# Onr/Council-GAN

Hardware: NVIDIA H100
Metric: training images/sec (gen+dis step) (higher is better)
Workload: dtype tf32

## Files before the change

### council_gan_b200/csrc/api.cu

```cuda
#include "common.cuh"
#include <string.h>

namespace cg {

static thread_local char g_err[512] = "";
std::atomic<uint64_t> g_launches{0};
thread_local int g_tc_mode = 7;
thread_local int g_pdl = 0;

void set_error(const char* fmt, ...) {
    va_list ap;
    va_start(ap, fmt);
    vsnprintf(g_err, sizeof(g_err), fmt, ap);
    va_end(ap);
}

int validate_geom(const cg_conv_geom& g) {
    CG_REQUIRE(g.G >= 1 && (g.x_groups == 1 || g.x_groups == g.G), "conv: x_groups=%d must be 1 or G=%d", g.x_groups, g.G);
    CG_REQUIRE(g.Cin % 4 == 0 && g.Cin > 0, "conv: Cin=%d must be a positive multiple of 4", g.Cin);
    CG_REQUIRE(g.Cout > 0 && g.B > 0 && g.H > 0 && g.W > 0, "conv: empty tensor");
    CG_REQUIRE(g.stride >= 1 && g.KH >= 1 && g.KW >= 1 && g.pad >= 0, "conv: bad kernel geometry");
    int Hin = g.ups ? 2 * g.H : g.H, Win = g.ups ? 2 * g.W : g.W;
    int Ho = (Hin + 2 * g.pad - g.KH) / g.stride + 1, Wo = (Win + 2 * g.pad - g.KW) / g.stride + 1;
    CG_REQUIRE(Ho == g.Ho && Wo == g.Wo, "conv: output size %dx%d inconsistent with geometry (expected %dx%d)", g.Ho, g.Wo, Ho, Wo);
// ... 52 lines not shown
    if (dir == 0) {
        if (i >= rows * K2p) return;
        long r = i / K2p;
        int k = (int)(i - r * K2p);
        dst[i] = k < K2 ? __ldg(src + r * K2 + k) : 0.f;
    } else {
        if (i >= rows * K2) return;
        long r = i / K2;
        int k = (int)(i - r * K2);
        dst[i] = __ldg(src + r * K2p + k);
    }
}
static int run_im2col(const cg_conv_geom& g, const float* x, float* P, cudaStream_t st) {
    cg_conv_geom p = patch_geom(g);
    long nimg = (long)(g.x_groups == 1 ? 1 : g.G) * g.B;
    long total4 = nimg * g.Ho * g.Wo * (p.Cin / 4);
    launch_k(im2col_small_kernel, cdiv(total4, 256), 256, 0, st, x, P, total4, g.H, g.W, g.Cin, g.Ho, g.Wo, g.KH, g.KW, g.stride, g.pad,
                                                          g.KH * g.KW * g.Cin, p.Cin);
    return check_launch("im2col_small");
}

}

using namespace cg;

extern "C" const char* cg_last_error(void) { return g_err; }

extern "C" int cg_device_info(int* sm_count, int* cc_major, int* cc_minor) {
    int dev = 0;
    cudaError_t e = cudaGetDevice(&dev);
    if (e != cudaSuccess) {
        set_error("cudaGetDevice: %s", cudaGetErrorString(e));
        return CG_ERR_NO_DEVICE;
    }
    cudaDeviceProp prop;
    e = cudaGetDeviceProperties(&prop, dev);
    if (e != cudaSuccess) {
        set_error("cudaGetDeviceProperties: %s", cudaGetErrorString(e));
        return CG_ERR_NO_DEVICE;
    }
    if (sm_count) *sm_count = prop.multiProcessorCount;
    if (cc_major) *cc_major = prop.major;
    if (cc_minor) *cc_minor = prop.minor;
    return prop.multiProcessorCount;
}

extern "C" int cg_set_tensor_core_mode(int mode) {
    int prev = g_tc_mode;
    g_tc_mode = mode == 1 ? 7 : (mode & 7);
    g_small_bn = ((mode >> 23) & 1) ? 0 : 1;
    g_wgrad_tma = ((mode >> 25) & 1) ? 0 : 1;
    g_pdl = (mode >> 22) & 1;
    g_tc_serial_epilogue = (mode >> 26) & 1;
    return prev;
}

extern "C" uint64_t cg_launch_count(void) { return g_launches.load(); }
extern "C" void cg_tensor_map_cache_stats(uint64_t* hits, uint64_t* misses) { tc_map_cache_stats(hits, misses); }

extern "C" int cg_zero(void* ptr, size_t bytes, void* stream) {
    cudaError_t e = cudaMemsetAsync(ptr, 0, bytes, (cudaStream_t)stream);
    if (e != cudaSuccess) {
        set_error("cg_zero: %s", cudaGetErrorString(e));
        return CG_ERR_CUDA;
    }
    return CG_OK;
}

extern "C" size_t cg_conv_workspace_bytes(const cg_conv_geom* g, int which) {
    if (!g) return 0;
    ConvDims d = conv_dims(*g);
    size_t need = 0;
    const bool patch_fwd = which == 0 && (g_tc_mode & 1) && patch_path(*g) && g->KH * g->KW >= 16;
    if (which == 2 && small_wgrad_supported(*g)) return small_ws(*g, 2);
    if (which == 1 && small_dgrad_supported(*g)) return small_ws(*g, 1);
    const bool patch_wgrad = which == 2 && (g_tc_mode & 4) && patch_path(*g);
    if (patch_fwd || patch_wgrad) {
        cg_conv_geom p = patch_geom(*g);
        ConvDims dp = conv_dims(p);
        size_t inner = which == 2 ? tc_wgrad_ws(p) : 0;
        size_t cs = which == 2 ? colsum_ws(g->G, dp.Mpix, g->Cout) : 0;
        if (cs > inner) inner = cs;
        need = patch_bytes(*g) + 2 * patch_w_bytes(*g) + inner;
        if (which == 2) return need;
    }
    if (which == 0 && (g_tc_mode & 1) && tc_fwd_supported(*g)) { size_t t = tc_fwd_ws(*g); need = t > need ? t : need; }
    if (which == 1) {
        if (g->ups) need = (size_t)g->G * g->B * d.Hin * d.Win * g->Cin * sizeof(float);
        if ((g_tc_mode & 2) && tc_dgrad_supported(*g)) { size_t t = tc_dgrad_ws(*g); need = t > need ? t : need; }
    }
    if (which == 2) {
        size_t a = ((g_tc_mode & 4) && tc_wgrad_supported(*g)) ? tc_wgrad_ws(*g) : simt_wgrad_ws(*g);
        size_t b = colsum_ws(g->G, d.Mpix, g->Cout);
        need = a > b ? a : b;
    }
    return need;
}

extern "C" int cg_conv_fwd(const cg_conv_geom* g, const float* x, const float* w, const float* bias, float* y, int act,
                           float slope, void* ws, size_t ws_bytes, void* stream) {
    if (int rc = validate_geom(*g)) return rc;
    cudaStream_t st = (cudaStream_t)stream;
    if (small_fwd_supported(*g, act)) return small_conv_fwd(*g, x, w, bias, y, st);
    if ((g_tc_mode & 1) && patch_path(*g) && g->KH * g->KW >= 16 && act != CG_ACT_TANH) {
        size_t need = cg_conv_workspace_bytes(g, 0);
        if (need > ws_bytes) {
// ... 108 lines not shown
```

### council_gan_b200/csrc/common.cuh

```cuda
#pragma once
#include <cuda.h>
#include <cuda_runtime.h>
#include <stdint.h>
#include <stdio.h>
#include <stdarg.h>
#include <atomic>
#include "../../include/council_b200.h"

namespace cg {

void set_error(const char* fmt, ...);
extern std::atomic<uint64_t> g_launches;
extern thread_local int g_tc_mode;
extern thread_local int g_small_bn;
extern thread_local int g_wgrad_tma;
extern thread_local int g_tc_serial_epilogue;

constexpr int CG_MAX_DEVICES = 64;
inline int current_device() {
    int dev = 0;
    cudaGetDevice(&dev);
    return dev >= 0 && dev < CG_MAX_DEVICES ? dev : 0;
}
struct PerDeviceOnce {
    std::atomic<bool> done[CG_MAX_DEVICES];
    bool first() { return !done[current_device()].exchange(true); }
    void reset() { done[current_device()].store(false); }
};

inline int check_launch(const char* what) {
    g_launches.fetch_add(1, std::memory_order_relaxed);
    cudaError_t e = cudaGetLastError();
    if (e != cudaSuccess) {
        set_error("%s: %s", what, cudaGetErrorString(e));
        return CG_ERR_CUDA;
    }
    return CG_OK;
}

#define CG_REQUIRE(cond, ...)                \
    do {                                     \
        if (!(cond)) {                       \
            cg::set_error(__VA_ARGS__);      \
            return CG_ERR_ARG;               \
        }                                    \
    } while (0)

static inline int cdiv(long a, long b) { return (int)((a + b - 1) / b); }

extern thread_local int g_pdl;
__device__ __forceinline__ void pdl_trigger() { asm volatile("griddepcontrol.launch_dependents;" ::: "memory"); }
__device__ __forceinline__ void pdl_wait() { asm volatile("griddepcontrol.wait;" ::: "memory"); }

template <typename... KArgs, typename... Args>
inline void launch_k(void (*kern)(KArgs...), dim3 grid, dim3 block, size_t smem, cudaStream_t st, Args&&... args) {
    cudaLaunchConfig_t cfg = {};
    cfg.gridDim = grid;
    cfg.blockDim = block;
    cfg.dynamicSmemBytes = smem;
    cfg.stream = st;
    cudaLaunchAttribute at[1];
    at[0].id = cudaLaunchAttributeProgrammaticStreamSerialization;
    at[0].val.programmaticStreamSerializationAllowed = g_pdl;
    cfg.attrs = at;
    cfg.numAttrs = 1;
    (void)cudaLaunchKernelEx(&cfg, kern, static_cast<KArgs>(args)...);
}

__device__ __forceinline__ float apply_act(float v, int act, float slope) {
// ... 63 lines not shown
```

### council_gan_b200/csrc/conv_tc.cu

```cuda
#include "common.cuh"
#include "tc_ptx.cuh"
#include <cstdlib>
#include <cstdio>
#include <cuda.h>
#include <mutex>
#include <string.h>

namespace cg {

typedef CUresult (*EncodeTiledFn)(CUtensorMap*, CUtensorMapDataType, cuuint32_t, void*, const cuuint64_t*, const cuuint64_t*,
                                  const cuuint32_t*, const cuuint32_t*, CUtensorMapInterleave, CUtensorMapSwizzle,
                                  CUtensorMapL2promotion, CUtensorMapFloatOOBfill);
typedef CUresult (*EncodeIm2colFn)(CUtensorMap*, CUtensorMapDataType, cuuint32_t, void*, const cuuint64_t*, const cuuint64_t*,
                                   const int*, const int*, cuuint32_t, cuuint32_t, const cuuint32_t*, CUtensorMapInterleave,
                                   CUtensorMapSwizzle, CUtensorMapL2promotion, CUtensorMapFloatOOBfill);
static EncodeTiledFn g_encode_tiled = nullptr;
static EncodeIm2colFn g_encode_im2col = nullptr;
static int g_sm_count_dev[CG_MAX_DEVICES] = {0};
static int sm_count_now() {
    int dev = current_device();
    if (!g_sm_count_dev[dev]) cudaDeviceGetAttribute(&g_sm_count_dev[dev], cudaDevAttrMultiProcessorCount, dev);
    return g_sm_count_dev[dev];
}
thread_local int g_small_bn = 1;
thread_local int g_tc_serial_epilogue = 0;
static int g_driver_version = 0;
static std::once_flag g_once;

struct MapKey {
    const void* ptr;
    int64_t a, b;
    int32_t v[8];
    bool operator==(const MapKey& o) const { return ptr == o.ptr && a == o.a && b == o.b && memcmp(v, o.v, sizeof(v)) == 0; }
};
struct MapSlot {
    MapKey key;
    CUtensorMap map;
    bool used;
};
constexpr int MAP_SLOTS = 8192;
static MapSlot* g_map_cache = nullptr;
static std::mutex g_map_mutex;
static std::atomic<uint64_t> g_map_hits{0}, g_map_misses{0};
static inline uint32_t map_hash(const MapKey& k) {
    uint64_t h = 1469598103934665603ull;
    const unsigned char* p = reinterpret_cast<const unsigned char*>(&k);
    for (size_t i = 0; i < sizeof(MapKey); i++) h = (h ^ p[i]) * 1099511628211ull;
    return (uint32_t)(h ^ (h >> 32)) & (MAP_SLOTS - 1);
}
template <class F>
static int cached_map(CUtensorMap* out, const MapKey& key, F encode) {
    const uint32_t slot = map_hash(key);
    {
        std::lock_guard<std::mutex> lock(g_map_mutex);
        if (!g_map_cache) g_map_cache = new MapSlot[MAP_SLOTS]();
        MapSlot& s = g_map_cache[slot];
        if (s.used && s.key == key) {
            *out = s.map;
            g_map_hits.fetch_add(1, std::memory_order_relaxed);
            return CG_OK;
        }
    }
    if (int rc = encode(out)) return rc;
    g_map_misses.fetch_add(1, std::memory_order_relaxed);
    std::lock_guard<std::mutex> lock(g_map_mutex);
    MapSlot& s = g_map_cache[slot];
    s.key = key;
    s.map = *out;
    s.used = true;
    return CG_OK;
}
void tc_map_cache_stats(uint64_t* hits, uint64_t* misses) {
    *hits = g_map_hits.load();
    *misses = g_map_misses.load();
}

static void init_driver() {
    std::call_once(g_once, [] {
        cudaDriverEntryPointQueryResult q;
        void* fn = nullptr;
        if (cudaGetDriverEntryPoint("cuTensorMapEncodeTiled", &fn, cudaEnableDefault, &q) == cudaSuccess && q == cudaDriverEntryPointSuccess)
            g_encode_tiled = (EncodeTiledFn)fn;
        fn = nullptr;
        if (cudaGetDriverEntryPoint("cuTensorMapEncodeIm2col", &fn, cudaEnableDefault, &q) == cudaSuccess && q == cudaDriverEntryPointSuccess)
            g_encode_im2col = (EncodeIm2colFn)fn;
        cudaDriverGetVersion(&g_driver_version);
    });
}

constexpr int TC_BM = 128;
constexpr int TC_BK = 32;
constexpr int TC_THREADS = 384;
constexpr int TC_MAX_STAGES = 12;
constexpr int TC_MAX_CLASSES = 4;

struct TcClass {
    CUtensorMap amap;
    int w0, h0;
    int out_h0, out_w0;
    int wrow_off;
    int pad_;
};
struct TcParams {
    CUtensorMap bmap;
    TcClass cls[TC_MAX_CLASSES];
    int ncls;
    int G, xg_images;
    int B, P, Q;
    int Cin, Cout, KH, KW, stride;
    int bn;
    int bk;
    int cps;
    int n_store;
    int out_H, out_W, out_sh, out_sw;
    int w_rows_per_group;
    float* y; const float* bias; const float* addend; const float* mask_src;
    float* stats;
    long stats_gbc;
    int act; float slope;
    int stages;
    int serial_epilogue;
};

__device__ __forceinline__ void tc_tile(const TcParams& p, int t, int MT, int NT, int& mt, int& nt, int& c, int& g) {
    if (p.serial_epilogue) {
        mt = t % MT;
        int r = t / MT;
        nt = r % NT;
        r /= NT;
        c = r % p.ncls;
        g = r / p.ncls;
        return;
    }
    c = t % p.ncls;
    int r = t / p.ncls;
    mt = r % MT;
    r /= MT;
    nt = r % NT;
    g = r / NT;
}

template <int BK, int BN>
__global__ void __launch_bounds__(TC_THREADS, 1) conv_tc_kernel(const __grid_constant__ TcParams p) {
    pdl_trigger();
    extern __shared__ __align__(1024) uint8_t smem_raw[];
    uint8_t* smem = reinterpret_cast<uint8_t*>((reinterpret_cast<uintptr_t>(smem_raw) + 1023) & ~(uintptr_t)1023);
    const int wg = __shfl_sync(0xffffffffu, threadIdx.x >> 7, 0), tid = threadIdx.x & 127;
    constexpr int a_bytes = TC_BM * BK * 4;
    constexpr int b_bytes = ((BN * BK * 4) + 1023) & ~1023;
    const int stage_bytes = p.cps * (a_bytes + b_bytes);
    constexpr int tx_chunk = a_bytes + BN * BK * 4;
    uint64_t* full_bar = reinterpret_cast<uint64_t*>(smem + (size_t)p.stages * stage_bytes);
    uint64_t* empty_bar = full_bar + p.stages;

    const int MT = (p.B * p.P * p.Q + TC_BM - 1) / TC_BM;
    const int NT = (p.Cout + BN - 1) / BN;
    const int tiles = p.G * p.ncls * NT * MT;
    const int kchunks = (p.Cin + BK - 1) / BK;
    const int kiters = p.KH * p.KW * kchunks;

    if (threadIdx.x == 0) {
        prefetch_tmap(&p.bmap);
        for (int c = 0; c < p.ncls; c++) prefetch_tmap(&p.cls[c].amap);
        for (int s = 0; s < p.stages; s++) {
            mbar_init(&full_bar[s], 1);
            mbar_init(&empty_bar[s], 2);
        }
        fence_barrier_init();
    }
    __syncthreads();
    pdl_wait();

    if (wg == 0) {
        if (tid == 0) {
            int stage = 0;
            uint32_t phase = 0;
            for (int t = blockIdx.x; t < tiles; t += gridDim.x) {
                int mt, nt, c, g;
                tc_tile(p, t, MT, NT, mt, nt, c, g);
                const TcClass& cl = p.cls[c];
                long m0 = (long)mt * TC_BM;
                int img = (int)(m0 / (p.P * p.Q));
                int rem = (int)(m0 - (long)img * p.P * p.Q);
                int pp = rem / p.Q, qq = rem - pp * p.Q;
                int n_coord = g * p.xg_images + img;
                int w_coord = cl.w0 + qq * p.stride;
                int h_coord = cl.h0 + pp * p.stride;
                int wrow = g * p.w_rows_per_group + cl.wrow_off + nt * BN;
                int kh = 0, kw = 0, kc = 0;
                for (int k0 = 0; k0 < kiters; k0 += p.cps) {
                    const int n = kiters - k0 < p.cps ? kiters - k0 : p.cps;
                    mbar_wait(&empty_bar[stage], phase ^ 1);
                    uint8_t* sa = smem + (size_t)stage * stage_bytes;
                    uint8_t* sb = sa + p.cps * a_bytes;
                    mbar_expect_tx(&full_bar[stage], (uint32_t)(n * tx_chunk));
                    for (int j = 0; j < n; j++) {
                        tma_load_im2col_4d(&cl.amap, &full_bar[stage], sa + j * a_bytes, kc * BK, w_coord, h_coord, n_coord, (uint16_t)kw,
                                           (uint16_t)kh);
                        tma_load_2d(&p.bmap, &full_bar[stage], sb + j * b_bytes, (kh * p.KW + kw) * p.Cin + kc * BK, wrow);
                        if (++kc == kchunks) { kc = 0; if (++kw == p.KW) { kw = 0; ++kh; } }
                    }
                    if (++stage == p.stages) { stage = 0; phase ^= 1; }
                }
            }
        }
        return;
    }

    const int cw = wg - 1;
    const int warp4 = tid >> 5, lane = tid & 31;
    const int row0 = cw * 64 + warp4 * 16 + (lane >> 2);
    const int cq = 2 * (lane & 3);
    const uint64_t desc0 = BK == 32 ? make_kmajor_sw128_desc(0) : make_kmajor_sw32_desc(0);
    float acc[BN / 2];
    int stage = 0;
    uint32_t phase = 0;
    for (int t = blockIdx.x; t < tiles; t += gridDim.x) {
        int mt, nt, c, g;
        tc_tile(p, t, MT, NT, mt, nt, c, g);
        const TcClass& cl = p.cls[c];
        int prev = -1;
        for (int k0 = 0; k0 < kiters; k0 += p.cps) {
            const int n = kiters - k0 < p.cps ? kiters - k0 : p.cps;
            mbar_wait(&full_bar[stage], phase);
            const uint32_t sa = smem_u32(smem + (size_t)stage * stage_bytes) + cw * (64 * BK * 4);
            const uint32_t sb = smem_u32(smem + (size_t)stage * stage_bytes) + p.cps * a_bytes;
            wgmma_fence();
            for (int j = 0; j < n; j++) {
                const uint64_t adesc = desc0 | (uint64_t)(((sa + j * a_bytes) & 0x3FFFF) >> 4);
                const uint64_t bdesc = desc0 | (uint64_t)(((sb + j * b_bytes) & 0x3FFFF) >> 4);
#pragma unroll
                for (int kk = 0; kk < BK / 8; kk++)
                    wgmma_tf32<BN>(acc, adesc + (uint64_t)(kk * 2), bdesc + (uint64_t)(kk * 2), (k0 | j | kk) != 0 ? 1 : 0);
            }
            wgmma_commit();
            wgmma_wait<1>();
            if (prev >= 0 && tid == 0) mbar_arrive(&empty_bar[prev]);
            prev = stage;
            if (++stage == p.stages) { stage = 0; phase ^= 1; }
        }
        wgmma_wait<0>();
        wgmma_reg_fence(acc, BN / 2);
        if (tid == 0) mbar_arrive(&empty_bar[prev]);

        const int pq = p.P * p.Q;
        long out_off[2];
        bool valid[2];
#pragma unroll
        for (int h = 0; h < 2; h++) {
            const int m = mt * TC_BM + row0 + 8 * h;
            valid[h] = m < p.B * pq;
            out_off[h] = 0;
            if (valid[h]) {
                int img = m / pq;
                int rem = m - img * pq;
                int pp = rem / p.Q, qq = rem - pp * p.Q;
                long pix = ((long)(g * p.B + img) * p.out_H + (pp * p.out_sh + cl.out_h0)) * p.out_W + (qq * p.out_sw + cl.out_w0);
                out_off[h] = pix * p.Cout + nt * p.n_store;
            }
        }
        if (p.stats) {
            const int tiles_per_img = pq / TC_BM;
            const int img = (mt * TC_BM) / pq;
            const int chunk = ((c * tiles_per_img + (mt - img * tiles_per_img)) << 3) + cw * 4 + warp4;
            const bool b2 = lane & 4, b3 = lane & 8;
            float* st = p.stats + ((long)chunk * p.stats_gbc + (long)(g * p.B + img) * p.Cout + nt * BN + cq) * 2 + (b3 ? 2 : 0) + (b2 ? 1 : 0);
#pragma unroll
            for (int j = 0; j < BN / 8; j++) {
                const float s0 = acc[4 * j] + acc[4 * j + 2], s1 = acc[4 * j + 1] + acc[4 * j + 3];
                const float q0 = acc[4 * j] * acc[4 * j] + acc[4 * j + 2] * acc[4 * j + 2];
                const float q1 = acc[4 * j + 1] * acc[4 * j + 1] + acc[4 * j + 3] * acc[4 * j + 3];
                const float k0 = b2 ? q0 : s0, k1 = b2 ? q1 : s1;
                const float r0 = __shfl_xor_sync(0xffffffffu, b2 ? s0 : q0, 4), r1 = __shfl_xor_sync(0xffffffffu, b2 ? s1 : q1, 4);
                const float x0 = k0 + r0, x1 = k1 + r1;
                float v = (b3 ? x1 : x0) + __shfl_xor_sync(0xffffffffu, b3 ? x0 : x1, 8);
                v += __shfl_xor_sync(0xffffffffu, v, 16);
                if (lane < 16) st[16 * j] = v;
            }
        }
        if (!(p.addend || p.mask_src) || p.serial_epilogue) {
#pragma unroll
            for (int j = 0; j < BN / 8; j++) {
                const int col = 8 * j + cq;
                if (col >= p.n_store) break;
                float2 bv = make_float2(0.f, 0.f);
                if (p.bias) bv = __ldg(reinterpret_cast<const float2*>(p.bias + (long)g * p.Cout + nt * p.n_store + col));
#pragma unroll
                for (int h = 0; h < 2; h++) {
                    if (!valid[h]) continue;
                    float2 o = make_float2(acc[4 * j + 2 * h] + bv.x, acc[4 * j + 2 * h + 1] + bv.y);
                    if (p.addend) {
                        const float2 a = __ldg(reinterpret_cast<const float2*>(p.addend + out_off[h] + col));
                        o.x += a.x; o.y += a.y;
                    }
                    if (p.mask_src) {
                        const float2 a = __ldg(reinterpret_cast<const float2*>(p.mask_src + out_off[h] + col));
                        o.x *= a.x > 0.f ? 1.f : p.slope; o.y *= a.y > 0.f ? 1.f : p.slope;
                    } else if (p.act != CG_ACT_NONE) {
                        o.x = apply_act(o.x, p.act, p.slope); o.y = apply_act(o.y, p.act, p.slope);
                    }
                    *reinterpret_cast<float2*>(p.y + out_off[h] + col) = o;
                }
            }
            continue;
        }
        constexpr int EB = BN == 256 ? 2 : BN / 8 < 8 ? BN / 8 : 8;
#pragma unroll
        for (int j0 = 0; j0 < BN / 8; j0 += EB) {
            float2 av[EB][2], mv[EB][2];
#pragma unroll
            for (int jj = 0; jj < EB; jj++) {
                const int col = 8 * (j0 + jj) + cq;
#pragma unroll
                for (int h = 0; h < 2; h++) {
                    const bool ld = col < p.n_store && valid[h];
                    av[jj][h] = p.addend && ld ? __ldg(reinterpret_cast<const float2*>(p.addend + out_off[h] + col)) : make_float2(0.f, 0.f);
                    mv[jj][h] = p.mask_src && ld ? __ldg(reinterpret_cast<const float2*>(p.mask_src + out_off[h] + col)) : make_float2(0.f, 0.f);
                }
            }
#pragma unroll
            for (int jj = 0; jj < EB; jj++) {
                const int j = j0 + jj, col = 8 * j + cq;
#pragma unroll
                for (int h = 0; h < 2; h++) {
                    if (col >= p.n_store || !valid[h]) continue;
                    float2 o = make_float2(acc[4 * j + 2 * h] + 0.f, acc[4 * j + 2 * h + 1] + 0.f);
                    if (p.addend) { o.x += av[jj][h].x; o.y += av[jj][h].y; }
                    if (p.mask_src) { o.x *= mv[jj][h].x > 0.f ? 1.f : p.slope; o.y *= mv[jj][h].y > 0.f ? 1.f : p.slope; }
                    *reinterpret_cast<float2*>(p.y + out_off[h] + col) = o;
                }
            }
        }
    }
}


static int encode_weights_map_raw(CUtensorMap* map, const float* w, long rows, long ktot, int bn, int bk) {
    cuuint64_t dims[2] = {(cuuint64_t)ktot, (cuuint64_t)rows};
    cuuint64_t strides[1] = {(cuuint64_t)ktot * 4};
    cuuint32_t box[2] = {(cuuint32_t)bk, (cuuint32_t)bn};
    cuuint32_t estr[2] = {1, 1};
    CUresult r = g_encode_tiled(map, CU_TENSOR_MAP_DATA_TYPE_TFLOAT32, 2, (void*)w, dims, strides, box, estr,
                                CU_TENSOR_MAP_INTERLEAVE_NONE, bk == 32 ? CU_TENSOR_MAP_SWIZZLE_128B : CU_TENSOR_MAP_SWIZZLE_32B,
                                CU_TENSOR_MAP_L2_PROMOTION_L2_256B, CU_TENSOR_MAP_FLOAT_OOB_FILL_NONE);
    if (r != CUDA_SUCCESS) {
        set_error("cuTensorMapEncodeTiled(weights rows=%ld ktot=%ld bn=%d) failed: %d", rows, ktot, bn, (int)r);
        return CG_ERR_CUDA;
    }
    return CG_OK;
}

static int encode_weights_map(CUtensorMap* map, const float* w, long rows, long ktot, int bn, int bk = TC_BK) {
    MapKey k{};
    k.ptr = w; k.a = rows; k.b = ktot; k.v[0] = bn; k.v[1] = bk; k.v[7] = 1;
    return cached_map(map, k, [&](CUtensorMap* m) { return encode_weights_map_raw(m, w, rows, ktot, bn, bk); });
}

static int encode_weights_map_p(TcParams& p, const float* w, long rows, long ktot) {
    return encode_weights_map(&p.bmap, w, rows, ktot, p.bn, p.bk);
}

static int encode_act_map_raw(CUtensorMap* map, const float* x, long N, int H, int W, int C, int lo_w, int lo_h, int up_w, int up_h,
                              int stride, int bk) {
    cuuint64_t dims[4] = {(cuuint64_t)C, (cuuint64_t)W, (cuuint64_t)H, (cuuint64_t)N};
    cuuint64_t strides[3] = {(cuuint64_t)C * 4, (cuuint64_t)W * C * 4, (cuuint64_t)H * W * C * 4};
    int lower[2] = {lo_w, lo_h};
    int upper[2] = {up_w, up_h};
    cuuint32_t estr[4] = {1, (cuuint32_t)stride, (cuuint32_t)stride, 1};
    CUresult r = g_encode_im2col(map, CU_TENSOR_MAP_DATA_TYPE_TFLOAT32, 4, (void*)x, dims, strides, lower, upper, bk, TC_BM, estr,
                                 CU_TENSOR_MAP_INTERLEAVE_NONE, bk == 32 ? CU_TENSOR_MAP_SWIZZLE_128B : CU_TENSOR_MAP_SWIZZLE_32B,
                                 CU_TENSOR_MAP_L2_PROMOTION_L2_128B, CU_TENSOR_MAP_FLOAT_OOB_FILL_NONE);
    if (r != CUDA_SUCCESS) {
        set_error("cuTensorMapEncodeIm2col(N=%ld H=%d W=%d C=%d corners %d,%d / %d,%d stride %d) failed: %d", N, H, W, C, lo_w, lo_h,
                  up_w, up_h, stride, (int)r);
        return CG_ERR_CUDA;
    }
    if (g_driver_version <= 13010 && (long)N * H * W * C * 4 < 131072) reinterpret_cast<uint64_t*>(map)[1] &= ~(1ull << 21);
    return CG_OK;
}

static int encode_act_map(CUtensorMap* map, const float* x, long N, int H, int W, int C, int lo_w, int lo_h, int up_w, int up_h,
                          int stride, int bk = TC_BK) {
    MapKey k{};
    k.ptr = x; k.a = N; k.b = ((int64_t)H << 32) | (uint32_t)W;
    k.v[0] = C; k.v[1] = lo_w; k.v[2] = lo_h; k.v[3] = up_w; k.v[4] = up_h; k.v[5] = stride; k.v[6] = bk; k.v[7] = 2;
    return cached_map(map, k, [&](CUtensorMap* m) { return encode_act_map_raw(m, x, N, H, W, C, lo_w, lo_h, up_w, up_h, stride, bk); });
}

static int pick_bn(int cout) {
    if (cout % 256 == 0) return 256;
    if (cout == 128) return 128;
    if (cout == 64) return 64;
    if (cout <= 16 && cout % 4 == 0) return 16;
    return 0;
}
static int pick_bk(int cin) {
    if (cin % TC_BK == 0) return TC_BK;
    if (cin <= 16 && cin % 4 == 0) return 8;
    return 0;
}

static int fill_bn(int bn, long mpix, int groups_classes, int cout) {
    if (!g_small_bn) return bn;
    const int sms = sm_count_now();
    while (bn > 64 && cout % (bn / 2) == 0 && (long)groups_classes * cdiv(mpix, TC_BM) * (cout / bn) < sms) bn >>= 1;
    return bn;
}

bool tc_fwd_supported(const cg_conv_geom& g) {
    init_driver();
    if (!g_encode_tiled || !g_encode_im2col) return false;
    if (g.ups && !(g.KH == 3 && g.KW == 3 && g.stride == 1 && g.pad == 1 && g.Cin % TC_BK == 0)) return false;
    if (pick_bk(g.Cin) == 0) return false;
    if (pick_bn(g.Cout) == 0) return false;
    if (g.pad > 120 || g.KH > 120) return false;
    if ((long)g.B * (g.ups ? g.H * g.W : g.Ho * g.Wo) < TC_BM) return false;
    return true;
}

template <int BK>
static void (*tc_kernel_for(int bn))(TcParams) {
    switch (bn) {
        case 16: return conv_tc_kernel<BK, 16>;
        case 64: return conv_tc_kernel<BK, 64>;
        case 128: return conv_tc_kernel<BK, 128>;
        case 256: return conv_tc_kernel<BK, 256>;
    }
    return nullptr;
}

static int launch_tc(TcParams& p, cudaStream_t st) {
    int a_bytes = TC_BM * p.bk * 4, b_bytes = ((p.bn * p.bk * 4) + 1023) & ~1023;
    int chunk_bytes = a_bytes + b_bytes;
    int kiters = p.KH * p.KW * ((p.Cin + p.bk - 1) / p.bk);
    int cps = p.bn <= 128 ? 2 : 1;
    if (p.bk == 8) cps = 8;
    while (cps > 1 && (cps > kiters || cps * chunk_bytes > 64 * 1024)) cps >>= 1;
    p.cps = cps;
    int stage_bytes = cps * chunk_bytes;
    int stages = (226 * 1024 - 1024 - 2 * TC_MAX_STAGES * 8) / stage_bytes;
    if (stages > TC_MAX_STAGES) stages = TC_MAX_STAGES;
    if (stages > 4 && stage_bytes >= 48 * 1024) stages = 4;
    if (p.n_store == 0) p.n_store = p.bn;
    p.stages = stages;
    p.serial_epilogue = g_tc_serial_epilogue;
    size_t smem = (size_t)stages * stage_bytes + 1024  + 2 * stages * 8;
    void (*kern)(TcParams) = p.bk == 32 ? tc_kernel_for<32>(p.bn) : tc_kernel_for<8>(p.bn);
    if (!kern) {
        set_error("conv_tc: no kernel for N tile %d / K chunk %d", p.bn, p.bk);
        return CG_ERR_ARG;
    }
    static PerDeviceOnce attr_set;
    if (attr_set.first()) {
        for (int bn : {16, 64, 128, 256}) {
            cudaError_t e = cudaFuncSetAttribute(tc_kernel_for<32>(bn), cudaFuncAttributeMaxDynamicSharedMemorySize, 227 * 1024);
            if (e == cudaSuccess) e = cudaFuncSetAttribute(tc_kernel_for<8>(bn), cudaFuncAttributeMaxDynamicSharedMemorySize, 227 * 1024);
            if (e != cudaSuccess) {
                attr_set.reset();
                set_error("cudaFuncSetAttribute(conv_tc_kernel): %s", cudaGetErrorString(e));
                return CG_ERR_CUDA;
            }
        }
    }
    int MT = cdiv((long)p.B * p.P * p.Q, TC_BM);
    long tiles = (long)p.G * p.ncls * ((p.Cout + p.bn - 1) / p.bn) * MT;
    const long slots = sm_count_now();
    int grid = (int)(tiles < slots ? tiles : slots);
    launch_k(kern, grid, TC_THREADS, smem, st, p);
    return check_launch("conv_tc_kernel");
}


__global__ void ups_weight_transform_kernel(const float* __restrict__ w, float* __restrict__ wc, long total, int Cout, int Cin) {
    pdl_trigger();
    pdl_wait();
    long i = (long)blockIdx.x * blockDim.x + threadIdx.x;
    if (i >= total) return;
    int ci = (int)(i % Cin);
    long t = i / Cin;
    int ss = (int)(t % 2); t /= 2;
    int r = (int)(t % 2); t /= 2;
    int co = (int)(t % Cout); t /= Cout;
    int cls = (int)(t % 4);
    int g = (int)(t / 4);
    int a = cls >> 1, b = cls & 1;
    int kh0 = a == 0 ? (r == 0 ? 0 : 1) : (r == 0 ? 0 : 2), kh1 = a == 0 ? (r == 0 ? 0 : 2) : (r == 0 ? 1 : 2);
    int kw0 = b == 0 ? (ss == 0 ? 0 : 1) : (ss == 0 ? 0 : 2), kw1 = b == 0 ? (ss == 0 ? 0 : 2) : (ss == 0 ? 1 : 2);
    const float* wp = w + ((long)g * Cout + co) * 9 * Cin + ci;
    float acc = 0.f;
    for (int kh = kh0; kh <= kh1; kh++)
        for (int kw = kw0; kw <= kw1; kw++) acc += __ldg(wp + (kh * 3 + kw) * Cin);
    wc[i] = acc;
}

size_t tc_fwd_ws(const cg_conv_geom& g) {
    return g.ups ? (size_t)g.G * 4 * g.Cout * 4 * g.Cin * sizeof(float) : 0;
}

int tc_fwd_stats_chunks(const cg_conv_geom& g) {
// ... 695 lines not shown
```

### council_gan_b200/csrc/tc_ptx.cuh

```cuda
#pragma once
#include <cuda.h>
#include <cuda_runtime.h>
#include <stdint.h>

namespace cg {

__device__ __forceinline__ uint32_t smem_u32(const void* p) { return (uint32_t)__cvta_generic_to_shared(p); }

__device__ __forceinline__ void mbar_init(uint64_t* bar, uint32_t count) {
    asm volatile("mbarrier.init.shared::cta.b64 [%0], %1;" ::"r"(smem_u32(bar)), "r"(count));
}
__device__ __forceinline__ void mbar_expect_tx(uint64_t* bar, uint32_t bytes) {
    asm volatile("mbarrier.arrive.expect_tx.shared::cta.b64 _, [%0], %1;" ::"r"(smem_u32(bar)), "r"(bytes) : "memory");
}
__device__ __forceinline__ void mbar_arrive(uint64_t* bar) {
    asm volatile("mbarrier.arrive.shared::cta.b64 _, [%0];" ::"r"(smem_u32(bar)) : "memory");
}
__device__ __forceinline__ void mbar_wait(uint64_t* bar, uint32_t parity) {
    uint32_t done;
    const uint32_t addr = smem_u32(bar);
    do {
        asm volatile(
            "{\n"
            ".reg .pred p;\n"
            "mbarrier.try_wait.parity.shared::cta.b64 p, [%1], %2;\n"
            "selp.u32 %0, 1, 0, p;\n"
            "}\n"
            : "=r"(done)
            : "r"(addr), "r"(parity)
            : "memory");
    } while (!done);
}
__device__ __forceinline__ void fence_barrier_init() { asm volatile("fence.mbarrier_init.release.cluster;" ::: "memory"); }
__device__ __forceinline__ void fence_proxy_async() { asm volatile("fence.proxy.async.shared::cta;" ::: "memory"); }

__device__ __forceinline__ void tma_load_2d(const CUtensorMap* map, uint64_t* bar, void* dst, int c0, int c1) {
    asm volatile(
        "cp.async.bulk.tensor.2d.shared::cluster.global.mbarrier::complete_tx::bytes [%0], [%1, {%3, %4}], [%2];" ::"r"(smem_u32(dst)),
        "l"(map), "r"(smem_u32(bar)), "r"(c0), "r"(c1)
        : "memory");
}
__device__ __forceinline__ void tma_load_im2col_4d(const CUtensorMap* map, uint64_t* bar, void* dst, int c, int w, int h, int n,
                                                   uint16_t off_w, uint16_t off_h) {
    asm volatile(
        "cp.async.bulk.tensor.4d.shared::cluster.global.im2col.mbarrier::complete_tx::bytes [%0], [%1, {%3, %4, %5, %6}], [%2], {%7, %8};" ::
            "r"(smem_u32(dst)),
        "l"(map), "r"(smem_u32(bar)), "r"(c), "r"(w), "r"(h), "r"(n), "h"(off_w), "h"(off_h)
        : "memory");
}
__device__ __forceinline__ void tma_load_4d(const CUtensorMap* map, uint64_t* bar, void* dst, int c0, int c1, int c2, int c3) {
    asm volatile(
        "cp.async.bulk.tensor.4d.shared::cluster.global.mbarrier::complete_tx::bytes [%0], [%1, {%3, %4, %5, %6}], [%2];" ::"r"(smem_u32(dst)),
        "l"(map), "r"(smem_u32(bar)), "r"(c0), "r"(c1), "r"(c2), "r"(c3)
        : "memory");
}
__device__ __forceinline__ void tma_load_5d(const CUtensorMap* map, uint64_t* bar, void* dst, int c0, int c1, int c2, int c3, int c4) {
    asm volatile(
        "cp.async.bulk.tensor.5d.shared::cluster.global.mbarrier::complete_tx::bytes [%0], [%1, {%3, %4, %5, %6, %7}], [%2];" ::"r"(smem_u32(dst)),
        "l"(map), "r"(smem_u32(bar)), "r"(c0), "r"(c1), "r"(c2), "r"(c3), "r"(c4)
        : "memory");
}
__device__ __forceinline__ void prefetch_tmap(const CUtensorMap* map) {
    asm volatile("prefetch.tensormap [%0];" ::"l"(map) : "memory");
}

__device__ __forceinline__ uint64_t make_kmajor_sw128_desc(uint32_t smem_addr) {
    uint64_t d = 0;
    d |= (uint64_t)((smem_addr & 0x3FFFF) >> 4);
    d |= (uint64_t)1 << 16;
    d |= (uint64_t)(1024 >> 4) << 32;
    d |= (uint64_t)1 << 62;
    return d;
}
__device__ __forceinline__ uint64_t make_kmajor_sw32_desc(uint32_t smem_addr) {
    uint64_t d = 0;
    d |= (uint64_t)((smem_addr & 0x3FFFF) >> 4);
    d |= (uint64_t)1 << 16;
    d |= (uint64_t)(256 >> 4) << 32;
    d |= (uint64_t)3 << 62;
    return d;
}

__device__ __forceinline__ void wgmma_fence() { asm volatile("wgmma.fence.sync.aligned;" ::: "memory"); }
__device__ __forceinline__ void wgmma_commit() { asm volatile("wgmma.commit_group.sync.aligned;" ::: "memory"); }
template <int N>
__device__ __forceinline__ void wgmma_wait() { asm volatile("wgmma.wait_group.sync.aligned %0;" ::"n"(N) : "memory"); }
__device__ __forceinline__ void wgmma_reg_fence(float* d, int n) {
    for (int i = 0; i < n; i++) asm volatile("" : "+f"(d[i])::"memory");
}

template <int N>
__device__ __forceinline__ void wgmma_tf32(float* d, uint64_t adesc, uint64_t bdesc, int scale_d);
template <> __device__ __forceinline__ void wgmma_tf32<16>(float* d, uint64_t adesc, uint64_t bdesc, int scale_d) {
    asm volatile(
        "{\n.reg .pred p;\nsetp.ne.b32 p, %10, 0;\n"
        "wgmma.mma_async.sync.aligned.m64n16k8.f32.tf32.tf32 {%0, %1, %2, %3, %4, %5, %6, %7}, %8, %9, p, 1, 1;\n}\n"
        : "+f"(d[0]), "+f"(d[1]), "+f"(d[2]), "+f"(d[3]), "+f"(d[4]), "+f"(d[5]), "+f"(d[6]), "+f"(d[7])
        : "l"(adesc), "l"(bdesc), "r"(scale_d));
}
template <> __device__ __forceinline__ void wgmma_tf32<32>(float* d, uint64_t adesc, uint64_t bdesc, int scale_d) {
    asm volatile(
        "{\n.reg .pred p;\nsetp.ne.b32 p, %18, 0;\n"
        "wgmma.mma_async.sync.aligned.m64n32k8.f32.tf32.tf32 {%0, %1, %2, %3, %4, %5, %6, %7, %8, %9, %10, %11, %12, %13, %14, %15}, %16, %17, p, 1, 1;\n}\n"
        : "+f"(d[0]), "+f"(d[1]), "+f"(d[2]), "+f"(d[3]), "+f"(d[4]), "+f"(d[5]), "+f"(d[6]), "+f"(d[7]), "+f"(d[8]), "+f"(d[9]), "+f"(d[10]), "+f"(d[11]), "+f"(d[12]), "+f"(d[13]), "+f"(d[14]), "+f"(d[15])
        : "l"(adesc), "l"(bdesc), "r"(scale_d));
}
template <> __device__ __forceinline__ void wgmma_tf32<64>(float* d, uint64_t adesc, uint64_t bdesc, int scale_d) {
    asm volatile(
        "{\n.reg .pred p;\nsetp.ne.b32 p, %34, 0;\n"
        "wgmma.mma_async.sync.aligned.m64n64k8.f32.tf32.tf32 {%0, %1, %2, %3, %4, %5, %6, %7, %8, %9, %10, %11, %12, %13, %14, %15, %16, %17, %18, %19, %20, %21, %22, %23, %24, %25, %26, %27, %28, %29, %30, %31}, %32, %33, p, 1, 1;\n}\n"
        : "+f"(d[0]), "+f"(d[1]), "+f"(d[2]), "+f"(d[3]), "+f"(d[4]), "+f"(d[5]), "+f"(d[6]), "+f"(d[7]), "+f"(d[8]), "+f"(d[9]), "+f"(d[10]), "+f"(d[11]), "+f"(d[12]), "+f"(d[13]), "+f"(d[14]), "+f"(d[15]), "+f"(d[16]), "+f"(d[17]), "+f"(d[18]), "+f"(d[19]), "+f"(d[20]), "+f"(d[21]), "+f"(d[22]), "+f"(d[23]), "+f"(d[24]), "+f"(d[25]), "+f"(d[26]), "+f"(d[27]), "+f"(d[28]), "+f"(d[29]), "+f"(d[30]), "+f"(d[31])
        : "l"(adesc), "l"(bdesc), "r"(scale_d));
}
template <> __device__ __forceinline__ void wgmma_tf32<128>(float* d, uint64_t adesc, uint64_t bdesc, int scale_d) {
// ... 48 lines not shown
```

Measured before the change: 45.88.

## Add TMA-based epilogue with producer-loaded addend/mask and bulk tensor stores

Adds a TMA epilogue path for the tensor-core conv kernel. A dedicated producer warp prefetches addend and mask tiles into swizzled shared-memory slots. Consumer warps apply bias, residual add, activation or mask in shared memory, and one thread issues 5D bulk tensor stores to global. The aim is to replace scattered per-thread global loads and stores with overlapped async bulk transfers. In exchange, the extra epilogue smem slots may reduce the number of pipeline stages, and cps is lowered for BN=128 tiles. Output tensor maps are cached and re-pointed with cuTensorMapReplaceAddress.

```diff
diff --git a/council_gan_b200/csrc/api.cu b/council_gan_b200/csrc/api.cu
--- a/council_gan_b200/csrc/api.cu
+++ b/council_gan_b200/csrc/api.cu
@@ -128,6 +128,7 @@
     g_wgrad_tma = ((mode >> 25) & 1) ? 0 : 1;
     g_pdl = (mode >> 22) & 1;
     g_tc_serial_epilogue = (mode >> 26) & 1;
+    g_tc_reg_epilogue = (mode >> 27) & 1;
     return prev;
 }
 
diff --git a/council_gan_b200/csrc/common.cuh b/council_gan_b200/csrc/common.cuh
--- a/council_gan_b200/csrc/common.cuh
+++ b/council_gan_b200/csrc/common.cuh
@@ -15,6 +15,7 @@
 extern thread_local int g_small_bn;
 extern thread_local int g_wgrad_tma;
 extern thread_local int g_tc_serial_epilogue;
+extern thread_local int g_tc_reg_epilogue;
 
 constexpr int CG_MAX_DEVICES = 64;
 inline int current_device() {
diff --git a/council_gan_b200/csrc/conv_tc.cu b/council_gan_b200/csrc/conv_tc.cu
--- a/council_gan_b200/csrc/conv_tc.cu
+++ b/council_gan_b200/csrc/conv_tc.cu
@@ -14,7 +14,9 @@
 typedef CUresult (*EncodeIm2colFn)(CUtensorMap*, CUtensorMapDataType, cuuint32_t, void*, const cuuint64_t*, const cuuint64_t*,
                                    const int*, const int*, cuuint32_t, cuuint32_t, const cuuint32_t*, CUtensorMapInterleave,
                                    CUtensorMapSwizzle, CUtensorMapL2promotion, CUtensorMapFloatOOBfill);
+typedef CUresult (*ReplaceAddressFn)(CUtensorMap*, void*);
 static EncodeTiledFn g_encode_tiled = nullptr;
+static ReplaceAddressFn g_replace_address = nullptr;
 static EncodeIm2colFn g_encode_im2col = nullptr;
 static int g_sm_count_dev[CG_MAX_DEVICES] = {0};
 static int sm_count_now() {
@@ -24,6 +26,7 @@
 }
 thread_local int g_small_bn = 1;
 thread_local int g_tc_serial_epilogue = 0;
+thread_local int g_tc_reg_epilogue = 0;
 static int g_driver_version = 0;
 static std::once_flag g_once;
 
@@ -84,6 +87,9 @@
         fn = nullptr;
         if (cudaGetDriverEntryPoint("cuTensorMapEncodeIm2col", &fn, cudaEnableDefault, &q) == cudaSuccess && q == cudaDriverEntryPointSuccess)
             g_encode_im2col = (EncodeIm2colFn)fn;
+        fn = nullptr;
+        if (cudaGetDriverEntryPoint("cuTensorMapReplaceAddress", &fn, cudaEnableDefault, &q) == cudaSuccess && q == cudaDriverEntryPointSuccess)
+            g_replace_address = (ReplaceAddressFn)fn;
         cudaDriverGetVersion(&g_driver_version);
     });
 }
@@ -120,6 +126,8 @@
     int act; float slope;
     int stages;
     int serial_epilogue;
+    CUtensorMap ymap, addmap, maskmap;
+    int epi_slots, epi_slot_bytes;
 };
 
 __device__ __forceinline__ void tc_tile(const TcParams& p, int t, int MT, int NT, int& mt, int& nt, int& c, int& g) {
@@ -138,6 +146,15 @@
     r /= MT;
     nt = r % NT;
     g = r / NT;
+}
+
+__device__ __forceinline__ void tc_half_coords(const TcParams& p, int g, int mt, int h, int& q, int& n) {
+    const int pq = p.P * p.Q;
+    const int m = mt * TC_BM + 64 * h;
+    const int img = m / pq, rem = m - img * pq;
+    const int pp = rem / p.Q;
+    q = rem - pp * p.Q;
+    n = (g * p.B + img) * (p.out_H / p.out_sh) + pp;
 }
 
 template <int BK, int BN>
@@ -150,8 +167,13 @@
     constexpr int b_bytes = ((BN * BK * 4) + 1023) & ~1023;
     const int stage_bytes = p.cps * (a_bytes + b_bytes);
     constexpr int tx_chunk = a_bytes + BN * BK * 4;
-    uint64_t* full_bar = reinterpret_cast<uint64_t*>(smem + (size_t)p.stages * stage_bytes);
+    constexpr bool tma_epi = BK == 32 && BN >= 64;
+    const int epi_slots = tma_epi ? p.epi_slots : 0;
+    uint8_t* epi = smem + (size_t)p.stages * stage_bytes;
+    uint64_t* full_bar = reinterpret_cast<uint64_t*>(epi + (size_t)epi_slots * p.epi_slot_bytes);
     uint64_t* empty_bar = full_bar + p.stages;
+    uint64_t* efull_bar = empty_bar + p.stages;
+    uint64_t* eempty_bar = efull_bar + epi_slots;
 
     const int MT = (p.B * p.P * p.Q + TC_BM - 1) / TC_BM;
     const int NT = (p.Cout + BN - 1) / BN;
@@ -165,6 +187,15 @@
         for (int s = 0; s < p.stages; s++) {
             mbar_init(&full_bar[s], 1);
             mbar_init(&empty_bar[s], 2);
+        }
+        if (epi_slots) {
+            prefetch_tmap(&p.ymap);
+            if (p.addend) prefetch_tmap(&p.addmap);
+            if (p.mask_src) prefetch_tmap(&p.maskmap);
+        }
+        for (int s = 0; s < epi_slots; s++) {
+            mbar_init(&efull_bar[s], 1);
+            mbar_init(&eempty_bar[s], 2);
         }
         fence_barrier_init();
     }
@@ -203,6 +234,35 @@
                     if (++stage == p.stages) { stage = 0; phase ^= 1; }
                 }
             }
+        } else if (tid == 32 && epi_slots) {
+            const uint32_t ebytes = (p.addend ? 2 * 8192 : 0) + (p.mask_src ? 2 * 8192 : 0);
+            int es = 0;
+            uint32_t ephase = 0;
+            for (int t = blockIdx.x; t < tiles; t += gridDim.x) {
+                int mt, nt, c, g;
+                tc_tile(p, t, MT, NT, mt, nt, c, g);
+                const TcClass& cl = p.cls[c];
+                int q[2], n[2];
+                tc_half_coords(p, g, mt, 0, q[0], n[0]);
+                tc_half_coords(p, g, mt, 1, q[1], n[1]);
+                for (int sl = 0; sl < BN / 32; sl++) {
+                    mbar_wait(&eempty_bar[es], ephase ^ 1);
+                    if (ebytes) {
+                        mbar_expect_tx(&efull_bar[es], ebytes);
+                        uint8_t* dst = epi + (size_t)es * p.epi_slot_bytes;
+                        const int c0 = nt * BN + 32 * sl;
+                        for (int h = 0; h < 2; h++) {
+                            if (p.addend) tma_load_5d(&p.addmap, &efull_bar[es], dst + h * 8192, c0, cl.out_w0, q[h], cl.out_h0, n[h]);
+                            if (p.mask_src)
+                                tma_load_5d(&p.maskmap, &efull_bar[es], dst + (p.addend ? 16384 : 0) + h * 8192, c0, cl.out_w0, q[h],
+                                            cl.out_h0, n[h]);
+                        }
+                    } else {
+                        mbar_arrive(&efull_bar[es]);
+                    }
+                    if (++es == epi_slots) { es = 0; ephase ^= 1; }
+                }
+            }
         }
         return;
     }
@@ -215,6 +275,8 @@
     float acc[BN / 2];
     int stage = 0;
     uint32_t phase = 0;
+    int es = 0;
+    uint32_t ephase = 0;
     for (int t = blockIdx.x; t < tiles; t += gridDim.x) {
         int mt, nt, c, g;
         tc_tile(p, t, MT, NT, mt, nt, c, g);
@@ -276,6 +338,61 @@
                 float v = (b3 ? x1 : x0) + __shfl_xor_sync(0xffffffffu, b3 ? x0 : x1, 8);
                 v += __shfl_xor_sync(0xffffffffu, v, 16);
                 if (lane < 16) st[16 * j] = v;
+            }
+        }
+        if constexpr (tma_epi) {
+            if (epi_slots) {
+                int q, n;
+                tc_half_coords(p, g, mt, cw, q, n);
+                const int r0 = warp4 * 16 + (lane >> 2);
+#pragma unroll
+                for (int sl = 0; sl < BN / 32; sl++) {
+                    float2 bv[4];
+#pragma unroll
+                    for (int jj = 0; jj < 4; jj++)
+                        bv[jj] = p.bias ? __ldg(reinterpret_cast<const float2*>(p.bias + (long)g * p.Cout + nt * BN + 32 * sl + 8 * jj + cq))
+                                        : make_float2(0.f, 0.f);
+                    mbar_wait(&efull_bar[es], ephase);
+                    uint8_t* half = epi + (size_t)es * p.epi_slot_bytes + cw * 8192;
+                    const uint8_t* msk = half + (p.addend ? 16384 : 0);
+#pragma unroll
+                    for (int jj = 0; jj < 4; jj++) {
+                        const int j = 4 * sl + jj;
+#pragma unroll
+                        for (int h = 0; h < 2; h++) {
+                            const int r = r0 + 8 * h;
+                            const int off = r * 128 + (((2 * jj + (cq >> 2)) ^ (r & 7)) << 4) + (cq & 3) * 4;
+                            float2 o = make_float2(acc[4 * j + 2 * h] + bv[jj].x, acc[4 * j + 2 * h + 1] + bv[jj].y);
+                            if (p.addend) {
+                                const float2 a = *reinterpret_cast<const float2*>(half + off);
+                                o.x += a.x; o.y += a.y;
+                            }
+                            if (p.mask_src) {
+                                const float2 a = *reinterpret_cast<const float2*>(msk + off);
+                                o.x *= a.x > 0.f ? 1.f : p.slope; o.y *= a.y > 0.f ? 1.f : p.slope;
+                            } else if (p.act != CG_ACT_NONE) {
+                                o.x = apply_act(o.x, p.act, p.slope); o.y = apply_act(o.y, p.act, p.slope);
+                            }
+                            *reinterpret_cast<float2*>(half + off) = o;
+                        }
+                    }
+                    fence_proxy_async();
+                    named_bar_sync(1 + cw, 128);
+                    if (tid == 0) {
+                        tma_store_5d(&p.ymap, half, nt * BN + 32 * sl, cl.out_w0, q, cl.out_h0, n);
+                        bulk_commit();
+                        if (sl > 0) {
+                            bulk_wait_read<1>();
+                            mbar_arrive(&eempty_bar[es == 0 ? epi_slots - 1 : es - 1]);
+                        }
+                        if (sl == BN / 32 - 1) {
+                            bulk_wait_read<0>();
+                            mbar_arrive(&eempty_bar[es]);
+                        }
+                    }
+                    if (++es == epi_slots) { es = 0; ephase ^= 1; }
+                }
+                continue;
             }
         }
         if (!(p.addend || p.mask_src) || p.serial_epilogue) {
@@ -332,6 +449,7 @@
             }
         }
     }
+    if (epi_slots && tid == 0) bulk_wait<0>();
 }
 
 
@@ -387,6 +505,32 @@
     return cached_map(map, k, [&](CUtensorMap* m) { return encode_act_map_raw(m, x, N, H, W, C, lo_w, lo_h, up_w, up_h, stride, bk); });
 }
 
+static int encode_out_map(CUtensorMap* map, const float* t, long NI, int H, int W, int C, int sh, int sw, int qbox) {
+    MapKey k{};
+    k.ptr = nullptr; k.a = NI; k.b = ((int64_t)H << 32) | (uint32_t)W;
+    k.v[0] = C; k.v[1] = sh; k.v[2] = sw; k.v[3] = qbox; k.v[7] = 3;
+    if (int rc = cached_map(map, k, [&](CUtensorMap* m) {
+            cuuint64_t dims[5] = {(cuuint64_t)C, (cuuint64_t)sw, (cuuint64_t)(W / sw), (cuuint64_t)sh, (cuuint64_t)(NI * H / sh)};
+            cuuint64_t strides[4] = {(cuuint64_t)C * 4, (cuuint64_t)sw * C * 4, (cuuint64_t)W * C * 4, (cuuint64_t)sh * W * C * 4};
+            cuuint32_t box[5] = {32, 1, (cuuint32_t)qbox, 1, (cuuint32_t)(64 / qbox)};
+            cuuint32_t estr[5] = {1, 1, 1, 1, 1};
+            CUresult r = g_encode_tiled(m, CU_TENSOR_MAP_DATA_TYPE_FLOAT32, 5, (void*)t, dims, strides, box, estr, CU_TENSOR_MAP_INTERLEAVE_NONE,
+                                        CU_TENSOR_MAP_SWIZZLE_128B, CU_TENSOR_MAP_L2_PROMOTION_L2_128B, CU_TENSOR_MAP_FLOAT_OOB_FILL_NONE);
+            if (r != CUDA_SUCCESS) {
+                set_error("cuTensorMapEncodeTiled(output NI=%ld H=%d W=%d C=%d strides %d,%d box q %d) failed: %d", NI, H, W, C, sh, sw, qbox, (int)r);
+                return CG_ERR_CUDA;
+            }
+            return CG_OK;
+        }))
+        return rc;
+    CUresult r = g_replace_address(map, (void*)t);
+    if (r != CUDA_SUCCESS) {
+        set_error("cuTensorMapReplaceAddress(output NI=%ld H=%d W=%d C=%d) failed: %d", NI, H, W, C, (int)r);
+        return CG_ERR_CUDA;
+    }
+    return CG_OK;
+}
+
 static int pick_bn(int cout) {
     if (cout % 256 == 0) return 256;
     if (cout == 128) return 128;
@@ -433,7 +577,7 @@
     int a_bytes = TC_BM * p.bk * 4, b_bytes = ((p.bn * p.bk * 4) + 1023) & ~1023;
     int chunk_bytes = a_bytes + b_bytes;
     int kiters = p.KH * p.KW * ((p.Cin + p.bk - 1) / p.bk);
-    int cps = p.bn <= 128 ? 2 : 1;
+    int cps = p.bn <= 64 ? 2 : 1;
     if (p.bk == 8) cps = 8;
     while (cps > 1 && (cps > kiters || cps * chunk_bytes > 64 * 1024)) cps >>= 1;
     p.cps = cps;
@@ -442,9 +586,30 @@
     if (stages > TC_MAX_STAGES) stages = TC_MAX_STAGES;
     if (stages > 4 && stage_bytes >= 48 * 1024) stages = 4;
     if (p.n_store == 0) p.n_store = p.bn;
+    p.serial_epilogue = g_tc_serial_epilogue;
+    p.epi_slots = 0;
+    const int nops = (p.addend ? 1 : 0) + (p.mask_src ? 1 : 0);
+    const bool aligned = ((uintptr_t)p.y | (uintptr_t)p.addend | (uintptr_t)p.mask_src) % 16 == 0;
+    if (g_replace_address && !g_tc_reg_epilogue && !p.serial_epilogue && p.bk == TC_BK && p.bn >= 64 && p.n_store == p.bn && (long)p.P * p.Q % TC_BM == 0 &&
+        (p.Q % 64 == 0 || 64 % p.Q == 0) && p.out_H % p.out_sh == 0 && p.out_W % p.out_sw == 0 && p.Cout % 4 == 0 && aligned) {
+        const int slot_bytes = (nops ? nops : 1) * 16384;
+        auto slots_beside = [&](int st) { return (int)((227L * 1024 - 1024 - (long)st * stage_bytes - 2 * st * 8) / (slot_bytes + 16)); };
+        while (slots_beside(stages) < 2 && stages > 4) stages--;
+        const int e = slots_beside(stages);
+        if (e >= 2) {
+            p.epi_slots = e < 4 ? e : 4;
+            p.epi_slot_bytes = slot_bytes;
+            const long ni = (long)p.G * p.B;
+            const int qbox = p.Q < 64 ? p.Q : 64;
+            if (int rc = encode_out_map(&p.ymap, p.y, ni, p.out_H, p.out_W, p.Cout, p.out_sh, p.out_sw, qbox)) return rc;
+            if (p.addend)
+                if (int rc = encode_out_map(&p.addmap, p.addend, ni, p.out_H, p.out_W, p.Cout, p.out_sh, p.out_sw, qbox)) return rc;
+            if (p.mask_src)
+                if (int rc = encode_out_map(&p.maskmap, p.mask_src, ni, p.out_H, p.out_W, p.Cout, p.out_sh, p.out_sw, qbox)) return rc;
+        }
+    }
     p.stages = stages;
-    p.serial_epilogue = g_tc_serial_epilogue;
-    size_t smem = (size_t)stages * stage_bytes + 1024  + 2 * stages * 8;
+    size_t smem = (size_t)stages * stage_bytes + 1024  + 2 * stages * 8 + (size_t)p.epi_slots * (p.epi_slot_bytes + 16);
     void (*kern)(TcParams) = p.bk == 32 ? tc_kernel_for<32>(p.bn) : tc_kernel_for<8>(p.bn);
     if (!kern) {
         set_error("conv_tc: no kernel for N tile %d / K chunk %d", p.bn, p.bk);
diff --git a/council_gan_b200/csrc/tc_ptx.cuh b/council_gan_b200/csrc/tc_ptx.cuh
--- a/council_gan_b200/csrc/tc_ptx.cuh
+++ b/council_gan_b200/csrc/tc_ptx.cuh
@@ -60,6 +60,17 @@
         "l"(map), "r"(smem_u32(bar)), "r"(c0), "r"(c1), "r"(c2), "r"(c3), "r"(c4)
         : "memory");
 }
+__device__ __forceinline__ void tma_store_5d(const CUtensorMap* map, const void* src, int c0, int c1, int c2, int c3, int c4) {
+    asm volatile("cp.async.bulk.tensor.5d.global.shared::cta.tile.bulk_group [%0, {%2, %3, %4, %5, %6}], [%1];" ::"l"(map),
+                 "r"(smem_u32(src)), "r"(c0), "r"(c1), "r"(c2), "r"(c3), "r"(c4)
+                 : "memory");
+}
+__device__ __forceinline__ void bulk_commit() { asm volatile("cp.async.bulk.commit_group;" ::: "memory"); }
+template <int N>
+__device__ __forceinline__ void bulk_wait_read() { asm volatile("cp.async.bulk.wait_group.read %0;" ::"n"(N) : "memory"); }
+template <int N>
+__device__ __forceinline__ void bulk_wait() { asm volatile("cp.async.bulk.wait_group %0;" ::"n"(N) : "memory"); }
+__device__ __forceinline__ void named_bar_sync(int id, int count) { asm volatile("bar.sync %0, %1;" ::"r"(id), "r"(count) : "memory"); }
 __device__ __forceinline__ void prefetch_tmap(const CUtensorMap* map) {
     asm volatile("prefetch.tensormap [%0];" ::"l"(map) : "memory");
 }
```

New measurement: 47.81, median of 6. 4.2% higher.
